# zz990099/foundationpose_cpp

Measured on AMD Instinct MI355X. Metric: pose-hypotheses/sec (Register N=252, 640x480), higher is better.
Workload: dtype f16; 1 GPU; Register N=252 hypotheses, 640x480 refine_itr=1, frame resident in HBM; mesh=synthetic ellipsoid V=2562 F=5120, 512x512 texture, weights=synthetic (seed 7), precision=f16 storage / f32 accumulate (the reference's TensorRT --fp16), parallelism=single GPU, collective=none

## Files before the change

### foundationpose_cpp_amd/csrc/fp_nn.hip

```cpp
#include "fp_nn.h"

#include <cmath>
#include <cstdio>
#include <cstdlib>
#include <cstring>
#include <algorithm>
#include <map>
#include <atomic>
#include <memory>
#include <thread>
#include <utility>

namespace fp {

typedef _Float16 h8 __attribute__((ext_vector_type(8)));
typedef _Float16 h4 __attribute__((ext_vector_type(4)));
typedef __bf16 b8 __attribute__((ext_vector_type(8)));
typedef __bf16 b4 __attribute__((ext_vector_type(4)));
typedef float f4 __attribute__((ext_vector_type(4)));
typedef int i2 __attribute__((ext_vector_type(2)));
typedef int i4 __attribute__((ext_vector_type(4)));
typedef int i8 __attribute__((ext_vector_type(8)));

static constexpr int EMBED = 512, HEADS = 4, HDIM = 128;
// ... 1034 lines not shown
  return 0;
}


struct Ctx {
  hipStream_t s;
  Profiler *prof;
  const Net *net;
  NNScratch *ws = nullptr;
};

#ifdef FP_TEST_HOOKS
#define FP_HOOK static int
static unsigned long long *g_clk_probe = nullptr;
static NNScratch g_hook_ws;
#else
#define FP_HOOK [[maybe_unused]] static constexpr int
static constexpr unsigned long long *g_clk_probe = nullptr;
#endif
FP_HOOK g_conv_variant = 0;
FP_HOOK g_conv_ablate = 0;
FP_HOOK g_splitk_ablate = 0;
FP_HOOK g_i8_stream = 0;
FP_HOOK g_smallm = 1;
FP_HOOK g_enc_tail = 1;
FP_HOOK g_ln_pmean = 1;
FP_HOOK g_fuse_pose = 1;
FP_HOOK g_qkv_ablate = 0;
FP_HOOK g_att_variant = 1;

static constexpr int SPLITK_TARGET = 128;
static constexpr int SPLITK_MIN_KT = 9;
static constexpr int SMALL_DEEP_MAXKT = 18;
static constexpr int SMALLM_MAXKT = 80;
static constexpr int SMALLM_MAXT16 = 1024;


enum ConvKernel {
  CK_SMALLX, CK_SMALLM, CK_STEM_HALO, CK_GEMM_K32, CK_S2_HALO, CK_HALO, CK_HALO8, CK_PP32, CK_BIG_PP, CK_PP, CK_DEEP64, CK_DEEP128,
  CK_IGEMM128, CK_IGEMM64, CK_SPLITK_REDUCE
};

struct ConvProblem {
  int Cin = 0, Cout = 0, KH = 0, KW = 0, stride = 1, pad = 0, algo_K = 0;
  bool wfrag = false, wpack = false;
  int NB = 0, H = 0, W = 0, ipad = 0;
  int dt = DT_F16, odt = DT_F16;
  bool has_res = false;
  int split_imgs = 0;
  int grp_rows = 0;
  bool post = false;
  int conv_variant = 0, conv_ablate = 0, smallm = 1;
};

struct ConvStep {
  int kernel = 0;
  const char *name = "";
  int mi = 0, ni = 0;
  bool post = false;
  bool deep = false;
  bool wpack = false;
  int ablate = 0;
  int m_begin = 0, M = 0;
  int ksplit = 1, kt_per = 0;
  unsigned grid = 0;
  int block = 256, lds = 0;
  double flops = 0, bytes = 0;
};

struct ConvPlan {
  static constexpr int MAX_STEPS = 4;
  int n = 0;
  ConvStep step[MAX_STEPS];
  bool post_fused = false;
};

static void conv_out_hw(int KH, int KW, int stride, int pad, int H, int W, int *OH, int *OW) {
  *OH = (H + 2 * pad - KH) / stride + 1;
  *OW = (W + 2 * pad - KW) / stride + 1;
  if (KH == 4 && pad == 2 && stride == 1) { *OH = H; *OW = W; }
}

static int plan_conv(const ConvProblem &q, ConvPlan *plan) {
  *plan = ConvPlan{};
  const bool B2 = !is_q8(q.dt);
  const bool SAME = q.dt == q.odt;
  const bool QOUT = odt_q(q.odt) >= 0;
  const bool grp = q.grp_rows > 0;
  int OH, OW;
  conv_out_hw(q.KH, q.KW, q.stride, q.pad, q.H, q.W, &OH, &OW);
  const int M = q.NB * OH * OW, Ktot = q.KH * q.KW * q.Cin, Cout = q.Cout;
  const int cin_b = q.Cin * elem_bytes(q.dt), KT = Ktot * elem_bytes(q.dt) / 128;
  double flops = 2.0 * (double)M * Cout * (q.algo_K > 0 ? q.algo_K : Ktot);
  double bytes = ((double)q.NB * q.H * q.W * q.Cin + (double)M * Cout * (q.has_res ? 2 : 1) + (double)Cout * Ktot) * elem_bytes(q.dt);
  constexpr int LDS_IG128 = 2 * (128 * 128 + 128 * 128), LDS_IG64 = 2 * (128 * 128 + 64 * 128);
  constexpr int LDS3_128 = 3 * (256 * 128 + 128 * 128);
  constexpr int LDS_BIG = 2 * (256 * 128 + 256 * 128);
  constexpr int LDS_HALO40 = ((10 * 42 + 7) / 8) * 1024 + 3 * 128 * 64;
  constexpr int LDS_HALO8 = ((10 * 42 + 7) / 8) * 1024 + 128 * 128;
  constexpr int LDS_STEM_HALO = ((11 * 84 + 15) / 16) * 1024 + 3 * 64 * 64;
  constexpr int LDS_DEEP64 = 6 * (64 + 128) * 128, LDS_DEEP128 = 4 * (128 + 128) * 128;
  constexpr int LDS_GEMM_K32 = 3 * (128 + 256) * 64;
  constexpr int LDS_S2_HALO = ((9 * 41 + 7) / 8) * 1024 + 3 * 128 * 64;
  constexpr int LDS_PP32 = 4 * (512 + 128) * 64;
  int m_begin = 0, ksplit = 1, kt_per = KT;
  bool overflow = false;
  const auto add = [&](int kernel, const char *name, int m_end, int grid, int block, int lds, double frac = 1.0) -> ConvStep & {
    overflow = overflow || plan->n == ConvPlan::MAX_STEPS;
    ConvStep &st = plan->step[overflow ? ConvPlan::MAX_STEPS - 1 : plan->n++];
    st = ConvStep{};
    st.kernel = kernel; st.name = name;
    st.m_begin = m_begin; st.M = m_end; st.ksplit = ksplit; st.kt_per = kt_per;
    st.grid = (unsigned)grid; st.block = block; st.lds = lds;
    st.flops = flops * frac; st.bytes = bytes * frac;
    flops *= (1.0 - frac); bytes *= (1.0 - frac);
    return st;
  };
  const auto finish = [&]() {
    FP_CHECK(!overflow, "plan_conv: more steps than ConvPlan holds");
    return 0;
// ... 54 lines not shown
      const int a = q.conv_ablate;
      add(CK_HALO, "conv_halo_kernel", M, grid, 256, LDS_HALO40).ablate = (q.dt == DT_F16 && (a == 1 || a == 2 || a == 8 || a == 16 || a == 32)) ? a : 0;
    } else {
      add(CK_HALO8, "conv_halo8_kernel", M, grid, 256, LDS_HALO8);
    }
    return finish();
  }
  if (B2 && !grp && (q.conv_variant == 0 || q.conv_variant == 8) && Cout == 128 && ksplit == 1 && KT >= 4 && KT <= 80) {
    const int mt_big = (M / 512 / 256) * 256;
    if (mt_big > 0) {
      add(CK_PP32, "conv_pp32_kernel<512,128>", mt_big * 512, mt_big, 512, LDS_PP32, (double)(mt_big * 512) / (double)M);
      m_begin = mt_big * 512;
      if (m_begin >= M) return finish();
    }
  }
  bool post_main = false;
  if (!(q.dt == DT_F16 && QOUT) && !grp && (q.conv_variant == 5 || q.conv_variant == 0 || q.conv_variant == 8) && Cout % 256 == 0 && ksplit == 1 && KT >= 2) {
    const int nt2 = Cout / 256;
    const int mt_all = M / 256;
    const int mt_big = (mt_all * nt2 / 256) * 256 / nt2;
    const int rows_left = M - mt_big * 256;
    post_main = q.post && !QOUT && mt_big > 0 && q.conv_variant == 0 && q.conv_ablate == 0 && KT >= 16 &&
                (rows_left == 0 || ((rows_left + 63) / 64) * (Cout / 128) <= 256);
    if (mt_big > 0) {
      const int a = q.conv_ablate;
      ConvStep &st = add(CK_BIG_PP, "conv_big_pp_kernel", mt_big * 256, mt_big * nt2, 512, LDS_BIG, (double)(mt_big * 256) / (double)M);
      st.ablate = (q.dt == DT_F16 && (a == 1 || a == 2 || a == 3 || a == 4 || a == 8 || a == 16)) ? a : 0;
      st.post = post_main;
      m_begin = mt_big * 256;
      if (m_begin >= M) { plan->post_fused = post_main; return finish(); }
    }
  }
  plan->post_fused = q.post && (post_main || ksplit > 1);
  if (!grp && (m_begin > 0 || M >= 8192 || small_deep) && (KT >= 16 || small_deep) && ksplit == 1 && Cout % 128 == 0) {
    const int n128 = Cout / 128;
    int rows = M - m_begin;
    if (((rows + 63) / 64) * n128 > 256) {
      const int mt_pp = (((rows + 255) / 256) * n128 / 256) * 256 / n128;
      const int rows_pp = std::min(mt_pp * 256, rows);
      const int rest = rows - rows_pp;
      const bool cascade = mt_pp > 0 && ((rest + 63) / 64) * n128 <= 256;
      const int m_end = cascade ? m_begin + rows_pp : M;
      add(CK_PP, "conv_pp_kernel(rem)", m_end, ((m_end - m_begin + 255) / 256) * n128, 512, LDS3_128, cascade ? (double)rows_pp / rows : 1.0);
      if (!cascade || rest == 0) return finish();
      m_begin += rows_pp;
      rows = rest;
// ... 445 lines not shown
  p.grp_rows = grp ? grp->rows : 0;
  p.in_shared = grp && grp->in_shared;
  p.res_shared = grp && grp->res_shared;
  p.grp_w_bytes = grp ? (unsigned)((size_t)L.Cout * L.KH * L.KW * L.Cin * es) : 0;
  FP_CHECK(!grp || (grp->rows % 128 == 0 && L.KH == 1 && L.KW == 1 && NB == 2 * grp->rows && !is_q8(L.dt)), "grouped launch: unsupported shape");
  p.in = (const unsigned char *)in.p; p.w = L.w; p.wfrag = L.wfrag; p.wpack = L.wpack; p.wpack128 = L.wpack128; p.wdeep = L.wdeep; p.bias = L.bias; p.cscale = is_q8(L.dt) ? L.cscale : nullptr;
  p.res = res ? (const unsigned char *)res->p : nullptr; p.out = (unsigned char *)out.p;
  p.out_dt = out.dt; p.res_dt = res ? res->dt : out.dt;
  p.NB = NB; p.H = H; p.W = W; p.Cin = L.Cin;
  p.KH = L.KH; p.KW = L.KW; p.stride = L.stride; p.pad = L.pad;
  p.ipad = ipad; p.opad = opad; p.rpad = rpad;
  conv_out_hw(L.KH, L.KW, L.stride, L.pad, H, W, &p.OH, &p.OW);
  p.Cout = L.Cout;
  p.M = NB * p.OH * p.OW;
  p.Ktot = L.KH * L.KW * L.Cin;
  p.cin_b = L.Cin * es;
  p.krow_b = p.Ktot * es;
  p.ntaps = L.KH * L.KW;
  p.relu = relu ? 1 : 0;
  p.split_imgs = split_imgs;
  p.out_ld = split_imgs > 0 ? 2 * L.Cout : L.Cout;
  p.res_ld = L.Cout;
  p.ksplit = 1; p.kt_per = p.krow_b / 128; p.partial = nullptr;
  p.m_begin = 0;
  FP_CHECK(ipad >= L.pad && (p.cin_b == 64 || p.cin_b % 128 == 0) && p.krow_b % 128 == 0 && (L.Cout % 64) == 0 &&
               (p.cin_b != 64 || L.KW % 2 == 0) && p.krow_b / 128 <= 80,
           "conv shape not supported by the MFMA kernel");
  {
    const int IWp = W + 2 * ipad;
    for (int kt = 0; kt < p.krow_b / 128; kt++) {
      int kh, kw, ch;
      if (p.cin_b >= 128) { ch = kt / p.ntaps; int tap = kt % p.ntaps; kh = tap / L.KW; kw = tap % L.KW; }
      else { ch = 0; int tap = 2 * kt; kh = tap / L.KW; kw = tap % L.KW; }
      p.koff[kt] = (unsigned)((kh * IWp + kw) * p.cin_b + ch * 128);
      if (2 * kt + 1 < 160) { p.koff32[2 * kt] = p.koff[kt]; p.koff32[2 * kt + 1] = p.koff[kt] + 64; }
    }
  }
  FP_CHECK(!res || res->dt == (rscale ? DT_I8 : is_q8(L.dt) ? DT_F16 : L.dt), "run_conv: the residual must have the layer's operand type (f16 for the 8-bit layers)");
  FP_CHECK(!post || (opad == 0 && split_imgs == 0 && !is_q8(out.dt) && post_fused), "run_conv: positional table on an unsupported layer");

  int odt = -1;
  ConvLaunch launch = nullptr;
#define FP_CONV_PAIR(DT_, ODT_) (odt = ODT_, launch = &launch_conv_step<DT_, ODT_>)
  if (out2) {
    if (L.dt == DT_FP8 && out2->dt == DT_FP8) FP_CONV_PAIR(DT_FP8, DT_DUAL_FP8);
    else if (L.dt == DT_I8 && out2->dt == DT_I8) FP_CONV_PAIR(DT_I8, DT_DUAL_I8);
    else if (L.dt == DT_F16 && out2->dt == DT_FP8) FP_CONV_PAIR(DT_F16, DT_DUAL_FP8);
// ... 12 lines not shown
      FP_CONV_PAIR(DT_F16, DT_QS_I8);
#else
      FP_CHECK(false, "run_conv: f16 -> scaled 8-bit alone exists in the test build only");
#endif
    } else FP_CONV_PAIR(DT_I8, DT_QS_I8);
  }
  else if (L.dt == DT_FP8 && out.dt == DT_FP8) FP_CONV_PAIR(DT_FP8, DT_FP8);
  else if (L.dt == DT_FP8 && out.dt == DT_F16) FP_CONV_PAIR(DT_FP8, DT_F16);
  else if (L.dt == DT_I8 && out.dt == DT_I8) FP_CONV_PAIR(DT_I8, DT_I8);
  else if (L.dt == DT_I8 && out.dt == DT_F16) FP_CONV_PAIR(DT_I8, DT_F16);
  else if (L.dt == DT_BF16 && out.dt == DT_BF16) FP_CONV_PAIR(DT_BF16, DT_BF16);
  else if (L.dt == DT_F16 && out.dt == DT_F16) FP_CONV_PAIR(DT_F16, DT_F16);
#undef FP_CONV_PAIR
  FP_CHECK(launch, "run_conv: unsupported combination of operand / output element types");

  ConvProblem q;
  q.Cin = L.Cin; q.Cout = L.Cout; q.KH = L.KH; q.KW = L.KW; q.stride = L.stride; q.pad = L.pad; q.algo_K = L.algo_K;
  q.wfrag = L.wfrag != nullptr; q.wpack = L.wpack != nullptr;
  q.NB = NB; q.H = H; q.W = W; q.ipad = ipad;
  q.dt = L.dt; q.odt = odt;
  q.has_res = res != nullptr; q.split_imgs = split_imgs;
  q.grp_rows = grp ? grp->rows : 0;
  q.post = post != nullptr;
  q.conv_variant = g_conv_variant; q.conv_ablate = g_conv_ablate; q.smallm = g_smallm;
  ConvPlan plan;
  if (plan_conv(q, &plan)) return 1;
  if (post_fused) *post_fused = plan.post_fused;
#ifdef FP_TEST_HOOKS
  g_last_conv_plan = plan; g_last_conv_odt = odt;
#endif
  for (int i = 0; i < plan.n; i++) {
    const ConvStep &st = plan.step[i];
    p.m_begin = st.m_begin; p.M = st.M;
    p.ksplit = st.ksplit; p.kt_per = st.kt_per;
    p.post = st.post ? (const unsigned char *)post : nullptr;
    if (st.ksplit > 1 && ensure_splitk(c, (size_t)st.ksplit * (st.M - st.m_begin) * L.Cout, &p.partial)) return 1;
    NetScope ps(c, tag, st);
    if (launch(c, st, p)) return 1;
  }
  return 0;
}

static int run_gemm(const Ctx &c, const char *tag, const ConvLayer &L, const void *in, int rows, void *out, bool relu,
                    const void *res = nullptr, const ConvGroup *grp = nullptr) {
  Act ai{const_cast<void *>(in), L.dt, 1.f}, ao{out, L.dt, 1.f}, ar{const_cast<void *>(res), L.dt, 1.f};
  return run_conv(c, tag, L, ai, rows, 1, 1, 0, ao, 0, relu, res ? &ar : nullptr, 0, 0, grp);
}

template <int DT>
struct DtTag {
  static constexpr int value = DT;
  using E = typename ElemT<DT>::t;
};
template <typename F>
static void with_dt(int dt, F &&f) {
  if (dt == DT_BF16) f(DtTag<DT_BF16>{});
// ... 718 lines not shown
```

### foundationpose_cpp_amd/csrc/fp_nn_conv_kernels.inc

```


__device__ __forceinline__ void glds16_asm(const void *gsrc, unsigned lds_addr) {
  unsigned keep;
  asm volatile("s_mov_b32 %0, m0\n\ts_mov_b32 m0, %2\n\ts_nop 0\n\tglobal_load_lds_dwordx4 %1, off\n\ts_mov_b32 m0, %0"
               : "=&s"(keep)
               : "v"(gsrc), "s"(lds_addr)
               : "memory");
}
__device__ __forceinline__ void glds16x2_asm(const void *gsrc, unsigned lds_addr) {
  unsigned keep;
  asm volatile("s_mov_b32 %0, m0\n\ts_mov_b32 m0, %2\n\ts_nop 0\n\tglobal_load_lds_dwordx4 %1, off\n\tglobal_load_lds_dwordx4 %1, off offset:1024\n\ts_mov_b32 m0, %0"
               : "=&s"(keep)
               : "v"(gsrc), "s"(lds_addr)
               : "memory");
}
__device__ __forceinline__ void glds16x4_asm(const void *gsrc, unsigned lds_addr) {
  unsigned keep;
  asm volatile("s_mov_b32 %0, m0\n\ts_mov_b32 m0, %2\n\ts_nop 0\n\tglobal_load_lds_dwordx4 %1, off\n\tglobal_load_lds_dwordx4 %1, off offset:1024\n\t"
               "global_load_lds_dwordx4 %1, off offset:2048\n\tglobal_load_lds_dwordx4 %1, off offset:3072\n\ts_mov_b32 m0, %0"
               : "=&s"(keep)
               : "v"(gsrc), "s"(lds_addr)
               : "memory");
}
#ifndef FP_X_NT
// ... 16 lines not shown
  const unsigned char *w;
  const unsigned char *wfrag;
  const unsigned char *wpack;
  const unsigned char *wpack128;
  const unsigned char *wdeep;
  const float *bias;
  const float *bias_img;
  const float *cscale;
  const unsigned char *res;
  unsigned char *out;
  unsigned char *out2;
  const float *rscale;
  const float *oinv;
  int NB, H, W, Cin, OH, OW, Cout, KH, KW, stride, pad;
  int ipad, opad, rpad;
  int M, Ktot, relu, out_ld, res_ld, split_imgs;
  int cin_b;
  int krow_b;
  int out_dt, res_dt;
  int ntaps;
  unsigned koff[80];
  unsigned koff32[160];
  int m_begin;
  int ksplit, kt_per;
  float *partial;
  int grp_rows, in_shared, res_shared;
  unsigned grp_w_bytes;
  unsigned long long *clk;
  const unsigned char *post;
};

__device__ __forceinline__ int pack4_fp8(float a, float b, float c, float d) {
  int w = __builtin_amdgcn_cvt_pk_fp8_f32(sat_fp8(a), sat_fp8(b), 0, false);
  return __builtin_amdgcn_cvt_pk_fp8_f32(sat_fp8(c), sat_fp8(d), w, true);
}
__device__ __forceinline__ int pack4_u8(float a, float b, float c, float d) {
  unsigned w = __builtin_amdgcn_cvt_pk_u8_f32(__builtin_rintf(a), 0, 0u);
  w = __builtin_amdgcn_cvt_pk_u8_f32(__builtin_rintf(b), 1, w);
  w = __builtin_amdgcn_cvt_pk_u8_f32(__builtin_rintf(c), 2, w);
  w = __builtin_amdgcn_cvt_pk_u8_f32(__builtin_rintf(d), 3, w);
  return (int)(w ^ 0x80808080u);
}
template <int MI, int NI, int DT, int ODT, int EABL = 0, int NIT = NI, int NI0 = 0, class PixFn>
__device__ __forceinline__ void conv_epilogue_px(const ConvParams &p, f4 (&acc)[NIT][MI], int n_base, int lane, PixFn pix,
                                                 int bias_off = 0, int res_img_off = 0) {
  static_assert(NI == 4 || NI == 2, "wave covers 64 or 32 channels");
// ... 12 lines not shown
    float4 b0 = *reinterpret_cast<const float4 *>(p.bias + bias_off + nl + 32 * k), b1 = *reinterpret_cast<const float4 *>(p.bias + bias_off + nl + 32 * k + 4);
    bv[0] = b0.x; bv[1] = b0.y; bv[2] = b0.z; bv[3] = b0.w; bv[4] = b1.x; bv[5] = b1.y; bv[6] = b1.z; bv[7] = b1.w;
    if constexpr (DT == DT_I8) {
      if (p.bias_img) {
#pragma unroll
        for (int e = 0; e < 8; e++) bv[e] = 0.f;
      }
    }
    if constexpr (is_q8(DT)) {
      float4 s0 = *reinterpret_cast<const float4 *>(p.cscale + bias_off + nl + 32 * k), s1 = *reinterpret_cast<const float4 *>(p.cscale + bias_off + nl + 32 * k + 4);
      sc[0] = s0.x; sc[1] = s0.y; sc[2] = s0.z; sc[3] = s0.w; sc[4] = s1.x; sc[5] = s1.y; sc[6] = s1.z; sc[7] = s1.w;
    }
#pragma unroll
    for (int e = 0; e < 8; e++) {
      const int jj = (NI == 4) ? 2 * k + (e >> 2) : (e >> 1);
      const int ni = (NI == 4) ? (e & 3) : (e & 1);
#pragma unroll
      for (int mi = 0; mi < MI; mi++) {
        if constexpr (DT == DT_I8) acc[NI0 + ni][mi][jj] = __builtin_fmaf((float)__float_as_int(acc[NI0 + ni][mi][jj]), sc[e], bv[e]);
        else if constexpr (DT == DT_FP8) acc[NI0 + ni][mi][jj] = __builtin_fmaf(acc[NI0 + ni][mi][jj], sc[e], bv[e]);
        else acc[NI0 + ni][mi][jj] += bv[e];
      }
    }
  }
  float oi[SCALED ? NS : 1][8];
  if constexpr (SCALED) {
#pragma unroll
    for (int k = 0; k < NS; k++) {
      float4 s0 = *reinterpret_cast<const float4 *>(p.oinv + nl + 32 * k), s1 = *reinterpret_cast<const float4 *>(p.oinv + nl + 32 * k + 4);
      oi[k][0] = s0.x; oi[k][1] = s0.y; oi[k][2] = s0.z; oi[k][3] = s0.w; oi[k][4] = s1.x; oi[k][5] = s1.y; oi[k][6] = s1.z; oi[k][7] = s1.w;
    }
  }
  float rs[RQ ? NS : 1][8];
  if constexpr (RQ) {
#pragma unroll
    for (int k = 0; k < NS; k++) {
      float4 s0 = *reinterpret_cast<const float4 *>(p.rscale + nl + 32 * k), s1 = *reinterpret_cast<const float4 *>(p.rscale + nl + 32 * k + 4);
      rs[k][0] = s0.x; rs[k][1] = s0.y; rs[k][2] = s0.z; rs[k][3] = s0.w; rs[k][4] = s1.x; rs[k][5] = s1.y; rs[k][6] = s1.z; rs[k][7] = s1.w;
    }
  }
  constexpr bool POST = (EABL & 4) != 0;
  static_assert(!POST || (O16 >= 0 && !DUAL), "the positional table is added to plain 2-byte outputs");
  constexpr int GB = (POST || is_q8(DT)) ? (MI > 4 ? 4 : MI) : (MI > 8 ? (MI + 1) / 2 : MI);
#pragma unroll
  for (int g0 = 0; g0 < MI; g0 += GB) {
  size_t oofs[GB];
// ... 702 lines not shown
  } else {
    for (int kt = 0; kt < KT; kt++) {
      if (kt > 0) mfmas();
      FP_PP_BARRIER();
      ldfrags(rb);
      if (kt + 2 < KT) {
        stage(kt + 2, wb3);
        asm volatile("s_waitcnt vmcnt(%0)" ::"n"(G) : "memory");
      } else {
        asm volatile("s_waitcnt vmcnt(0)" ::: "memory");
      }
      asm volatile("s_waitcnt lgkmcnt(0)" ::: "memory");
      FP_PP_BARRIER();
      rb = (rb == 2) ? 0 : rb + 1;
      wb3 = (wb3 == 2) ? 0 : wb3 + 1;
    }
    mfmas();
  }
#undef FP_PP_BARRIER

  conv_epilogue<4, NREP, DT, ODT>(p, acc, m0 + grp * 128 + wm * 64, n0 + wn * (BN / 2), lane);
}

template <int ABL, int DT, int ODT = DT, bool POST = false, bool LSTORE = false>
__global__ __launch_bounds__(512, 2) void conv_big_pp_kernel(const ConvParams p) {
  extern __shared__ __attribute__((aligned(16))) unsigned char smem[];
  constexpr int BM = 256, BN = 256;
  constexpr int XB = BM * 128, WB = BN * 128, STAGE = XB + WB;
  constexpr int MI = 8, NI = 4;

  const int tid = threadIdx.x, lane = tid & 63;
  const int wave = __builtin_amdgcn_readfirstlane(tid >> 6);
  const int wm = wave >> 2, wn = wave & 3;
  const int n_tiles = p.Cout / BN;
  int logical;
  {
    const int nblk = gridDim.x, b = blockIdx.x;
    const int xcd = b & 7, within = b >> 3, q = nblk >> 3, r = nblk & 7;
    logical = (xcd < r ? xcd * (q + 1) : r * (q + 1) + (xcd - r) * q) + within;
  }
  const int mt = logical / n_tiles, nt = logical - mt * n_tiles;
  const int m0 = mt * BM, n0 = nt * BN;
  const int ohw = p.OH * p.OW;
  const int IHp = p.H + 2 * p.ipad, IWp = p.W + 2 * p.ipad;

  const int srow = lane >> 3;
  const int g = (lane & 7) ^ srow;
  unsigned xoff[4], woffv[4];
#pragma unroll
  for (int i = 0; i < 4; i++) {
    int m = min(m0 + (wave * 4 + i) * 8 + srow, p.M - 1);
    int img = m / ohw;
    int rem = m - img * ohw;
    int oh = rem / p.OW, ow = rem - oh * p.OW;
    int ih0 = oh * p.stride - p.pad + p.ipad, iw0 = ow * p.stride - p.pad + p.ipad;
    xoff[i] = (unsigned)(((img * IHp + ih0) * IWp + iw0) * p.cin_b + g * 16);
    int row = (wave * 4 + i) * 8 + srow;
    woffv[i] = (unsigned)((n0 + row) * p.krow_b + g * 16);
  }
  const unsigned char *in_b = p.in;
  const unsigned char *w_b = p.w;
  const unsigned lds_base = (unsigned)(size_t)(__attribute__((address_space(3))) unsigned char *)smem;

  auto stage_x = [&](int kt, int buf) {
    const unsigned xs = lds_base + buf * STAGE;
    const unsigned char *xb = in_b + p.koff[kt];
#pragma unroll
    for (int i = 0; i < 4; i++) glds16_asm(xb + xoff[i], xs + (wave * 4 + i) * 1024);
  };
  const bool packed = p.wpack128 != nullptr;
  const unsigned char *wpk = p.wpack128 + ((size_t)nt * (p.krow_b >> 7) * 8 + wave) * 4096 + lane * 16;
  auto stage_w = [&](int kt, int buf) {
    const unsigned ws = lds_base + buf * STAGE + XB;
    if (packed) { glds16x4_asm(wpk + (size_t)kt * 32768, ws + wave * 4096); return; }
    const unsigned char *wb = w_b + (size_t)kt * 128;
#pragma unroll
    for (int i = 0; i < 4; i++) glds16_asm(wb + woffv[i], ws + (wave * 4 + i) * 1024);
  };

  f4 acc[NI][MI];
#pragma unroll
  for (int a = 0; a < NI; a++)
#pragma unroll
    for (int b = 0; b < MI; b++) acc[a][b] = (f4){0.f, 0.f, 0.f, 0.f};

  const int frow = lane & 15, fk = lane >> 4;
  int xfo[2], wfo[2];
#pragma unroll
  for (int ks = 0; ks < 2; ks++) {
    int slot = (ks * 4 + fk) ^ (lane & 7);
    xfo[ks] = (wm * 128 + frow) * 128 + slot * 16;
    wfo[ks] = XB + (wn * 64 + frow) * 128 + slot * 16;
  }

#define FP_BAR()                         \
  do {                                   \
    __builtin_amdgcn_s_barrier();        \
    asm volatile("" ::: "memory");      \
    __builtin_amdgcn_sched_barrier(0);   \
  } while (0)
#define FP_LGKM0() asm volatile("s_waitcnt lgkmcnt(0)" ::: "memory")
#define FP_VM0() asm volatile("s_waitcnt vmcnt(0)" ::: "memory")
#define FP_PP_LOOP(LD0, LD1, MF0, MF1)                                   \
  do {                                                                   \
    const int KT = p.krow_b >> 7;                                        \
    stage_x(0, 0);                                                       \
    stage_w(0, 0);                                                       \
    FP_VM0();                                                            \
    FP_BAR();                                                            \
    if (p.clk && tid == 0) { p.clk[blockIdx.x * 4] = __builtin_readcyclecounter(); p.clk[blockIdx.x * 4 + 1] = wall_clock64(); } \
    int buf = 0;                                                         \
    if (wm == 0) {                                                       \
      for (int kt = 0; kt < KT; kt++) {                                  \
        LD0(buf);                                                        \
// ... 80 lines not shown
      __builtin_amdgcn_s_setprio(1);
#pragma unroll
      for (int ni = 0; ni < NI; ni++)
#pragma unroll
        for (int mi = 0; mi < MI; mi++)
          acc[ni][mi] = mfma32<DT>(wf[ni], xf[mi], acc[ni][mi]);
      __builtin_amdgcn_s_setprio(0);
    };
    FP_PP_LOOP(ld0, ld1, mf, mf);
  }
#undef FP_PP_LOOP
#undef FP_BAR
#undef FP_LGKM0
#undef FP_VM0
  if (p.clk && tid == 0) { p.clk[blockIdx.x * 4 + 2] = __builtin_readcyclecounter(); p.clk[blockIdx.x * 4 + 3] = wall_clock64(); }

  if (ABL & 4) {
#pragma unroll
    for (int a = 0; a < NI; a++)
#pragma unroll
      for (int b = 0; b < MI; b++) asm volatile("" ::"v"(acc[a][b]));
    return;
  }
  if constexpr (LSTORE && ABL == 0 && !POST && !is_q8(DT) && odt_q(ODT) < 0) {
    __syncthreads();
    conv_epilogue_lds<MI, NI, DT, ODT, 4>(p, acc, m0 + wm * 128, n0 + wn * 64, lane, smem + wave * (4 * 16 * 128 + 4 * 64));
    return;
  }
  conv_epilogue<MI, NI, DT, ODT, ((ABL >> 3) & 3) | (POST ? 4 : 0)>(p, acc, m0 + wm * 128, n0 + wn * 64, lane);
}

template <int BM, int BN, int DT, int ODT = DT>
__global__ __launch_bounds__(512, 2) void conv_pp32_kernel(const ConvParams p) {
  extern __shared__ __attribute__((aligned(16))) unsigned char smem[];
  constexpr int WM = BM / 128, WN = BN / 64;
  static_assert(WM * WN == 8, "8 waves");
  constexpr int XP = BM / 16, WP = BN / 16, PER = (XP + WP) / 8;
  constexpr int XB = XP * 1024, STAGE = (XP + WP) * 1024;
  constexpr int MI = 8, NI = 4;

  const int tid = threadIdx.x, lane = tid & 63;
  const int wave = __builtin_amdgcn_readfirstlane(tid >> 6);
  const int grp = wave >> 2;
  const int wm = wave / WN, wn = wave - wm * WN;
  const int n_tiles = p.Cout / BN;
  int logical;
  {
    const int nblk = gridDim.x, b = blockIdx.x;
    const int xcd = b & 7, within = b >> 3, q = nblk >> 3, r = nblk & 7;
    logical = (xcd < r ? xcd * (q + 1) : r * (q + 1) + (xcd - r) * q) + within;
  }
  const int mt = logical / n_tiles, nt = logical - mt * n_tiles;
// ... 985 lines not shown
```

### foundationpose_cpp_amd/csrc/fp_nn_test_hooks.inc

```

__global__ __launch_bounds__(256) void mfma_peak_kernel(float *out, int iters, int zero_operands, unsigned long long *clk) {
  using fp::f4;
  using fp::h8;
  const int lane = threadIdx.x & 63;
  h8 a, b;
  unsigned st = 2654435761u * (unsigned)(blockIdx.x * 256 + threadIdx.x + 1);
#pragma unroll
  for (int i = 0; i < 8; i++) {
    st = st * 1664525u + 1013904223u;
    a[i] = (_Float16)(((st >> 8) & 0xffff) / 65536.0f - 0.5f);
    st = st * 1664525u + 1013904223u;
    b[i] = (_Float16)(((st >> 8) & 0xffff) / 65536.0f - 0.5f);
    if (zero_operands) { a[i] = 0; b[i] = 0; }
  }
  unsigned long long c0 = 0, w0 = 0;
  if (clk && blockIdx.x == 0 && threadIdx.x == 0) { c0 = __builtin_readcyclecounter(); w0 = wall_clock64(); }
  f4 acc[8];
#pragma unroll
  for (int j = 0; j < 8; j++) acc[j] = (f4){0.f, 0.f, 0.f, 0.f};
  for (int i = 0; i < iters; i++) {
#pragma unroll
    for (int j = 0; j < 8; j++)
      asm volatile("v_mfma_f32_16x16x32_f16 %0, %1, %2, %0" : "+v"(acc[j]) : "v"(a), "v"(b));
  }
// ... 90 lines not shown
  fp::ConvLayer L;
  L.Cout = Cout; L.Cin = Cin; L.ntaps = ntaps;
  L.rows_f32.assign(rows, rows + (size_t)Cout * ntaps * Cin);
  std::vector<float> sw, tm;
  std::vector<double> qsum;
  const auto q = fp::quantise_q8(L, fp::DT_I8, s_in, &sw, &qsum, m_int, J, &tm);
  std::memcpy(q_out, q.data(), q.size());
  std::memcpy(sw_out, sw.data(), sw.size() * sizeof(float));
  std::memcpy(tmat_t_out, tm.data(), tm.size() * sizeof(float));
  return 0;
}
int fpt_quantise_q8(int dt, const float *rows, int Cout, int ntaps, int Cin, const float *s_in, unsigned char *q_out, float *sw_out) {
  if (!fp::is_q8(dt) || !rows || !s_in || !q_out || !sw_out || Cout < 1 || ntaps < 1 || Cin < 1) return 1;
  fp::ConvLayer L;
  L.Cout = Cout; L.Cin = Cin; L.ntaps = ntaps;
  L.rows_f32.assign(rows, rows + (size_t)Cout * ntaps * Cin);
  std::vector<float> sw;
  std::vector<double> qsum;
  const auto q = fp::quantise_q8(L, dt, s_in, &sw, &qsum);
  std::memcpy(q_out, q.data(), q.size());
  std::memcpy(sw_out, sw.data(), sw.size() * sizeof(float));
  return 0;
}
int fpt_plan_conv(const int *shape10, int dt, int odt, int flags, int split_imgs, int grp_rows, int *fields11, char *names, int name_cap, int max, int *post_fused) {
  fp::ConvProblem q;
  q.Cin = shape10[0]; q.Cout = shape10[1]; q.KH = shape10[2]; q.KW = shape10[3]; q.stride = shape10[4]; q.pad = shape10[5];
  q.NB = shape10[6]; q.H = shape10[7]; q.W = shape10[8]; q.ipad = shape10[9];
  q.dt = dt; q.odt = odt;
  q.has_res = (flags & 1) != 0; q.post = (flags & 2) != 0; q.wfrag = (flags & 4) != 0; q.wpack = (flags & 8) != 0;
  q.split_imgs = split_imgs; q.grp_rows = grp_rows;
  q.conv_variant = fp::g_conv_variant; q.conv_ablate = fp::g_conv_ablate; q.smallm = fp::g_smallm;
  fp::ConvPlan plan;
  if (fp::plan_conv(q, &plan)) return -1;
  for (int i = 0; i < plan.n && i < max; i++) {
    const fp::ConvStep &st = plan.step[i];
    const int f[11] = {-1, -1, 0, st.m_begin, st.M, st.ksplit, st.post ? 1 : 0, st.kernel, st.kt_per, (int)st.grid, st.lds};
    std::memcpy(fields11 + (size_t)i * 11, f, sizeof(f));
    std::snprintf(names + (size_t)i * name_cap, (size_t)name_cap, "%s", st.name);
  }
  if (post_fused) *post_fused = plan.post_fused ? 1 : 0;
  return plan.n;
}
int fpt_plan_heads(int pass, int N, int dt, int fuse_offer, int *fields18, int *tail3) {
  fp::HeadsPlan p;
  if (fp::plan_heads(fp::heads_query(pass, N, dt, fuse_offer != 0), &p)) return 1;
  const fp::AttVariant &v = fp::ATT_VARIANTS[p.att.variant];
  const int f[18] = {p.qkv, p.qkv_ablate, (int)p.qkv_grid, p.qkv_lds, p.att.kernel, v.remap ? 1 : 0, v.ablate, p.att.B, p.att.T,
                     p.att.pitch, p.att.nq, (int)p.att.grid, p.att.block, p.att.lds, p.tail, p.pool, p.readout, p.fuse_pose ? 1 : 0};
  std::memcpy(fields18, f, sizeof(f));
  const int t[3] = {p.tail_tiles, (int)p.tail_grid, p.tail_lds};
  std::memcpy(tail3, t, sizeof(t));
  return 0;
}
void fpt_plan_track_window(const float *K9, float diameter, const float *poses16, int H, int W, int reach, int *out5, int n) {
  for (int i = 0; i < n; i++) {
    const fp::TrackWindow w = fp::plan_track_window(K9, diameter, poses16 + (size_t)i * 16, H, W, reach);
    const int f[5] = {w.kind, w.row0, w.row1, w.col0, w.col1};
    for (int k = 0; k < 5; k++) out5[(size_t)i * 5 + k] = f[k];
  }
}
void fpt_depth_filter_tile(int *tile_w, int *tile_h) { *tile_w = fp::DEPTH_FILTER_TILE_W; *tile_h = fp::DEPTH_FILTER_TILE_H; }
void fpt_set_conv_variant(int v) { fp::g_conv_variant = v; }
void fpt_set_i8_stream(int v) { fp::g_i8_stream = v; }
void fpt_set_q8_blocks(int v) { fp::g_q8_blocks = v & fp::Q8_BLOCKS_ALL; }
void fpt_set_conv_ablate(int v) { fp::g_conv_ablate = v; }
void fpt_set_splitk_ablate(int v) { fp::g_splitk_ablate = v; }

int fpt_clk_probe(int blocks, double *mhz_out, double *loop_cycles_out) {
  using namespace fp;
  if (blocks > 0) {
    if (g_clk_probe) (void)hipFree(g_clk_probe);
    FP_HIP_OK(hipMalloc((void **)&g_clk_probe, (size_t)blocks * 32));
    FP_HIP_OK(fp::memset_sync(g_clk_probe, 0, (size_t)blocks * 32));
    return 0;
  }
  FP_CHECK(g_clk_probe, "no probe");
  int n = -blocks;
  std::vector<unsigned long long> h((size_t)n * 4);
  FP_HIP_OK(hipDeviceSynchronize());
  FP_HIP_OK(fp::memcpy_sync(h.data(), g_clk_probe, h.size() * 8, hipMemcpyDeviceToHost));
  double sc = 0, sr = 0; int cnt = 0;
  for (int i = 0; i < n; i++) {
    if (h[i * 4 + 3] > h[i * 4 + 1]) { sc += (double)(h[i * 4 + 2] - h[i * 4]); sr += (double)(h[i * 4 + 3] - h[i * 4 + 1]); cnt++; }
  }
  if (mhz_out) *mhz_out = sr > 0 ? sc / sr * 100.0 : 0;
  if (loop_cycles_out) *loop_cycles_out = cnt ? sc / cnt : 0;
  (void)hipFree(g_clk_probe);
  g_clk_probe = nullptr;
  return 0;
}

int fpt_conv_dt(const float *x, const float *w, const float *bias, const float *res, int NB, int H, int W, int Cin, int Cout,
                int KH, int KW, int stride, int pad, int OH, int OW, int relu, int split_imgs, float *out, int iters,
                float *ms_out, int dt, int out_dt, float in_scale, float res_scale, float out_scale) {
  using namespace fp;
  const int ip = pad;
  const int Hp = H + 2 * ip, Wp = W + 2 * ip;
  const int es = elem_bytes(dt), oes = elem_bytes(out_dt);
  size_t nx = (size_t)NB * Hp * Wp * Cin, nw = (size_t)Cout * KH * KW * Cin;
  size_t M = (size_t)NB * OH * OW;
  size_t nout = M * Cout;
  DevBuf<unsigned char> dx(nx * es), dres(nout * es), dout(nout * 2 * oes);
  FP_CHECK(dx.p && dres.p && dout.p, "fpt_conv: allocation failed");
  std::vector<float> xp(nx, 0.f);
  for (int n = 0; n < NB; n++)
    for (int y = 0; y < H; y++)
      for (int xx = 0; xx < W; xx++)
        for (int c = 0; c < Cin; c++)
          xp[(((size_t)n * Hp + y + ip) * Wp + xx + ip) * Cin + c] = x[(((size_t)n * H + y) * W + xx) * Cin + c];
  auto hx = encode(xp.data(), nx, dt, in_scale);
  FP_HIP_OK(fp::memcpy_sync(dx.p, hx.data(), hx.size(), hipMemcpyHostToDevice));
  FP_HIP_OK(fp::memset_sync(dout.p, 0, nout * 2 * oes));
  if (res) {
    auto hr = encode(res, nout, dt, res_scale);
    FP_HIP_OK(fp::memcpy_sync(dres.p, hr.data(), hr.size(), hipMemcpyHostToDevice));
  }
  Net net;
  ConvLayer L;
  L.Cin = Cin; L.Cout = Cout; L.KH = KH; L.KW = KW; L.stride = stride; L.pad = pad;
  FP_CHECK(finish_layer(&net, std::vector<float>(w, w + nw), std::vector<float>(bias, bias + Cout), Cout, KH * KW, Cin, dt, &L), "fpt_conv: weight upload failed");
  FP_CHECK(!is_q8(dt) && !is_q8(out_dt), "fpt_conv_dt: 2-byte element types only (8-bit layers: fpt_conv_q8)");
  Ctx c{nullptr, nullptr, &net};
  (void)OH; (void)OW;
  const Act ain{dx.p, dt, in_scale}, aout{dout.p, out_dt, out_scale}, ares{dres.p, dt, res_scale};
  hipEvent_t e0, e1;
  FP_HIP_OK(hipEventCreate(&e0));
  FP_HIP_OK(hipEventCreate(&e1));
  if (run_conv(c, "t", L, ain, NB, H, W, ip, aout, 0, relu != 0, res ? &ares : nullptr, 0, split_imgs)) return 1;
  FP_HIP_OK(hipDeviceSynchronize());
  if (iters > 1) {
    FP_HIP_OK(hipEventRecord(e0, nullptr));
    for (int i = 0; i < iters; i++)
      if (run_conv(c, "t", L, ain, NB, H, W, ip, aout, 0, relu != 0, res ? &ares : nullptr, 0, split_imgs)) return 1;
    FP_HIP_OK(hipEventRecord(e1, nullptr));
    FP_HIP_OK(hipEventSynchronize(e1));
    float ms = 0;
    FP_HIP_OK(hipEventElapsedTime(&ms, e0, e1));
    if (ms_out) *ms_out = ms / iters;
  }
  (void)hipEventDestroy(e0);
  (void)hipEventDestroy(e1);
  std::vector<unsigned char> ho(nout * oes);
  FP_HIP_OK(fp::memcpy_sync(ho.data(), dout.p, ho.size(), hipMemcpyDeviceToHost));
  decode(ho.data(), nout, out_dt, out_scale, out);
  return 0;
}
int fpt_conv_q8(const float *x, const float *s_in, const float *w, const float *bias, const float *res, int NB, int H, int W, int Cin, int Cout,
                int KH, int KW, int stride, int pad, int OH, int OW, int relu, int split_imgs, int mode, const float *s_out, float *out16,
                float *outq, int iters, float *ms_out, int dt, float *wq_out, const float *s_res) {
  using namespace fp;
  FP_CHECK(is_q8(dt) && mode >= 0 && mode <= 5 && (mode < 4 || (dt == DT_I8 && res && s_res)), "fpt_conv_q8: invalid arguments");
  const int ip = pad, Hp = H + 2 * ip, Wp = W + 2 * ip;
  const size_t nx = (size_t)NB * Hp * Wp * Cin, nw = (size_t)Cout * KH * KW * Cin, M = (size_t)NB * OH * OW, nout = M * Cout;
  DevBuf<unsigned char> dx(nx), dres(nout * 2), d16(nout * 2), dq(nout);
  FP_CHECK(dx.p && dres.p && d16.p && dq.p, "fpt_conv_q8: allocation failed");
  std::vector<unsigned char> hx(nx, dt == DT_I8 ? 0x80 : 0x00);
  for (int n = 0; n < NB; n++)
    for (int y = 0; y < H; y++)
      for (int xx = 0; xx < W; xx++)
        for (int c = 0; c < Cin; c++) {
          const float v = x[(((size_t)n * H + y) * W + xx) * Cin + c] / s_in[c];
          unsigned char b;
          if (dt == DT_FP8) b = f32_to_e4m3_bits(v);
          else b = (unsigned char)((int)std::max(0.f, std::min(255.f, std::nearbyint(v))) ^ 0x80);
          hx[(((size_t)n * Hp + y + ip) * Wp + xx + ip) * Cin + c] = b;
        }
  FP_HIP_OK(fp::memcpy_sync(dx.p, hx.data(), nx, hipMemcpyHostToDevice));
// ... 637 lines not shown
```

Before: 23930 hypotheses/s.

## Absorb conv big-tile row remainder into taller 288-row tiles instead of a tail launch

When the big 256x256 conv path leaves leftover rows, the planner now spreads them over some blocks that use a 288-row (MI=9) tile, each taking an extra 32 rows, balanced across XCDs. The whole convolution then runs as one launch instead of a main kernel plus a separate tail kernel. The kernel body is templated on MI, and a ragged epilogue handles the partial tile. This adds LDS per block and register pressure for the tall variant, and the test harness gains guard bands to catch out-of-bounds writes.

```diff
diff --git a/foundationpose_cpp_amd/csrc/fp_nn.hip b/foundationpose_cpp_amd/csrc/fp_nn.hip
--- a/foundationpose_cpp_amd/csrc/fp_nn.hip
+++ b/foundationpose_cpp_amd/csrc/fp_nn.hip
@@ -1080,6 +1080,7 @@
 FP_HOOK g_conv_ablate = 0;
 FP_HOOK g_splitk_ablate = 0;
 FP_HOOK g_i8_stream = 0;
+FP_HOOK g_conv_ragged = 1;
 FP_HOOK g_smallm = 1;
 FP_HOOK g_enc_tail = 1;
 FP_HOOK g_ln_pmean = 1;
@@ -1109,6 +1110,7 @@
   int grp_rows = 0;
   bool post = false;
   int conv_variant = 0, conv_ablate = 0, smallm = 1;
+  int ragged = 1;
 };
 
 struct ConvStep {
@@ -1120,6 +1122,7 @@
   bool wpack = false;
   int ablate = 0;
   int m_begin = 0, M = 0;
+  int n_tall = 0;
   int ksplit = 1, kt_per = 0;
   unsigned grid = 0;
   int block = 256, lds = 0;
@@ -1154,6 +1157,7 @@
   constexpr int LDS_IG128 = 2 * (128 * 128 + 128 * 128), LDS_IG64 = 2 * (128 * 128 + 64 * 128);
   constexpr int LDS3_128 = 3 * (256 * 128 + 128 * 128);
   constexpr int LDS_BIG = 2 * (256 * 128 + 256 * 128);
+  constexpr int LDS_BIG_TALL = 2 * (288 * 128 + 256 * 128);
   constexpr int LDS_HALO40 = ((10 * 42 + 7) / 8) * 1024 + 3 * 128 * 64;
   constexpr int LDS_HALO8 = ((10 * 42 + 7) / 8) * 1024 + 128 * 128;
   constexpr int LDS_STEM_HALO = ((11 * 84 + 15) / 16) * 1024 + 3 * 64 * 64;
@@ -1254,6 +1258,12 @@
     const int rows_left = M - mt_big * 256;
     post_main = q.post && !QOUT && mt_big > 0 && q.conv_variant == 0 && q.conv_ablate == 0 && KT >= 16 &&
                 (rows_left == 0 || ((rows_left + 63) / 64) * (Cout / 128) <= 256);
+    const int n_tall = (rows_left + 31) / 32;
+    if (q.ragged && B2 && SAME && mt_big > 0 && rows_left > 0 && q.conv_variant == 0 && q.conv_ablate == 0 && !q.post && 256 % nt2 == 0 &&
+        n_tall * nt2 <= 256) {
+      add(CK_BIG_PP, "conv_big_pp_kernel", M, mt_big * nt2, 512, LDS_BIG_TALL).n_tall = n_tall;
+      return finish();
+    }
     if (mt_big > 0) {
       const int a = q.conv_ablate;
       ConvStep &st = add(CK_BIG_PP, "conv_big_pp_kernel", mt_big * 256, mt_big * nt2, 512, LDS_BIG, (double)(mt_big * 256) / (double)M);
@@ -1745,7 +1755,7 @@
   p.out_ld = split_imgs > 0 ? 2 * L.Cout : L.Cout;
   p.res_ld = L.Cout;
   p.ksplit = 1; p.kt_per = p.krow_b / 128; p.partial = nullptr;
-  p.m_begin = 0;
+  p.m_begin = 0; p.n_tall = 0;
   FP_CHECK(ipad >= L.pad && (p.cin_b == 64 || p.cin_b % 128 == 0) && p.krow_b % 128 == 0 && (L.Cout % 64) == 0 &&
                (p.cin_b != 64 || L.KW % 2 == 0) && p.krow_b / 128 <= 80,
            "conv shape not supported by the MFMA kernel");
@@ -1804,7 +1814,7 @@
   q.has_res = res != nullptr; q.split_imgs = split_imgs;
   q.grp_rows = grp ? grp->rows : 0;
   q.post = post != nullptr;
-  q.conv_variant = g_conv_variant; q.conv_ablate = g_conv_ablate; q.smallm = g_smallm;
+  q.conv_variant = g_conv_variant; q.conv_ablate = g_conv_ablate; q.smallm = g_smallm; q.ragged = g_conv_ragged;
   ConvPlan plan;
   if (plan_conv(q, &plan)) return 1;
   if (post_fused) *post_fused = plan.post_fused;
@@ -1813,7 +1823,7 @@
 #endif
   for (int i = 0; i < plan.n; i++) {
     const ConvStep &st = plan.step[i];
-    p.m_begin = st.m_begin; p.M = st.M;
+    p.m_begin = st.m_begin; p.M = st.M; p.n_tall = st.n_tall;
     p.ksplit = st.ksplit; p.kt_per = st.kt_per;
     p.post = st.post ? (const unsigned char *)post : nullptr;
     if (st.ksplit > 1 && ensure_splitk(c, (size_t)st.ksplit * (st.M - st.m_begin) * L.Cout, &p.partial)) return 1;
diff --git a/foundationpose_cpp_amd/csrc/fp_nn_conv_kernels.inc b/foundationpose_cpp_amd/csrc/fp_nn_conv_kernels.inc
--- a/foundationpose_cpp_amd/csrc/fp_nn_conv_kernels.inc
+++ b/foundationpose_cpp_amd/csrc/fp_nn_conv_kernels.inc
@@ -62,6 +62,7 @@
   unsigned koff[80];
   unsigned koff32[160];
   int m_begin;
+  int n_tall;
   int ksplit, kt_per;
   float *partial;
   int grp_rows, in_shared, res_shared;
@@ -120,6 +121,12 @@
         else acc[NI0 + ni][mi][jj] += bv[e];
       }
     }
+  }
+  if constexpr ((EABL & 8) != 0) {
+#pragma unroll
+    for (int a = 0; a < NI; a++)
+#pragma unroll
+      for (int b = 0; b < MI; b++) asm volatile("" : "+v"(acc[NI0 + a][b]));
   }
   float oi[SCALED ? NS : 1][8];
   if constexpr (SCALED) {
@@ -868,39 +875,35 @@
   conv_epilogue<4, NREP, DT, ODT>(p, acc, m0 + grp * 128 + wm * 64, n0 + wn * (BN / 2), lane);
 }
 
-template <int ABL, int DT, int ODT = DT, bool POST = false, bool LSTORE = false>
-__global__ __launch_bounds__(512, 2) void conv_big_pp_kernel(const ConvParams p) {
-  extern __shared__ __attribute__((aligned(16))) unsigned char smem[];
-  constexpr int BM = 256, BN = 256;
+template <int MI, int ABL, int DT, int ODT, bool POST, bool LSTORE>
+__device__ __forceinline__ void conv_big_pp_body(const ConvParams &p, unsigned char *smem, const int m0, const int nt) {
+  constexpr int BM = MI * 32, BN = 256;
   constexpr int XB = BM * 128, WB = BN * 128, STAGE = XB + WB;
-  constexpr int MI = 8, NI = 4;
+  constexpr int NI = 4;
+  constexpr int NPX = BM / 8, PLO = NPX / 8, PREM = NPX % 8, PHI = PLO + (PREM ? 1 : 0);
 
   const int tid = threadIdx.x, lane = tid & 63;
   const int wave = __builtin_amdgcn_readfirstlane(tid >> 6);
   const int wm = wave >> 2, wn = wave & 3;
-  const int n_tiles = p.Cout / BN;
-  int logical;
-  {
-    const int nblk = gridDim.x, b = blockIdx.x;
-    const int xcd = b & 7, within = b >> 3, q = nblk >> 3, r = nblk & 7;
-    logical = (xcd < r ? xcd * (q + 1) : r * (q + 1) + (xcd - r) * q) + within;
-  }
-  const int mt = logical / n_tiles, nt = logical - mt * n_tiles;
-  const int m0 = mt * BM, n0 = nt * BN;
+  const int n0 = nt * BN;
   const int ohw = p.OH * p.OW;
   const int IHp = p.H + 2 * p.ipad, IWp = p.W + 2 * p.ipad;
 
   const int srow = lane >> 3;
   const int g = (lane & 7) ^ srow;
-  unsigned xoff[4], woffv[4];
-#pragma unroll
-  for (int i = 0; i < 4; i++) {
-    int m = min(m0 + (wave * 4 + i) * 8 + srow, p.M - 1);
+  const int px0 = wave * PLO + min(wave, PREM);
+  unsigned xoff[PHI], woffv[4];
+#pragma unroll
+  for (int i = 0; i < PHI; i++) {
+    int m = min(m0 + (px0 + i) * 8 + srow, p.M - 1);
     int img = m / ohw;
     int rem = m - img * ohw;
     int oh = rem / p.OW, ow = rem - oh * p.OW;
     int ih0 = oh * p.stride - p.pad + p.ipad, iw0 = ow * p.stride - p.pad + p.ipad;
     xoff[i] = (unsigned)(((img * IHp + ih0) * IWp + iw0) * p.cin_b + g * 16);
+  }
+#pragma unroll
+  for (int i = 0; i < 4; i++) {
     int row = (wave * 4 + i) * 8 + srow;
     woffv[i] = (unsigned)((n0 + row) * p.krow_b + g * 16);
   }
@@ -912,7 +915,8 @@
     const unsigned xs = lds_base + buf * STAGE;
     const unsigned char *xb = in_b + p.koff[kt];
 #pragma unroll
-    for (int i = 0; i < 4; i++) glds16_asm(xb + xoff[i], xs + (wave * 4 + i) * 1024);
+    for (int i = 0; i < PHI; i++)
+      if (i < PLO || wave < PREM) glds16_asm(xb + xoff[i], xs + (px0 + i) * 1024);
   };
   const bool packed = p.wpack128 != nullptr;
   const unsigned char *wpk = p.wpack128 + ((size_t)nt * (p.krow_b >> 7) * 8 + wave) * 4096 + lane * 16;
@@ -935,7 +939,7 @@
 #pragma unroll
   for (int ks = 0; ks < 2; ks++) {
     int slot = (ks * 4 + fk) ^ (lane & 7);
-    xfo[ks] = (wm * 128 + frow) * 128 + slot * 16;
+    xfo[ks] = (wm * (MI * 16) + frow) * 128 + slot * 16;
     wfo[ks] = XB + (wn * 64 + frow) * 128 + slot * 16;
   }
 
@@ -1062,12 +1066,38 @@
       for (int b = 0; b < MI; b++) asm volatile("" ::"v"(acc[a][b]));
     return;
   }
-  if constexpr (LSTORE && ABL == 0 && !POST && !is_q8(DT) && odt_q(ODT) < 0) {
+  if constexpr (LSTORE && MI == 8 && ABL == 0 && !POST && !is_q8(DT) && odt_q(ODT) < 0) {
     __syncthreads();
     conv_epilogue_lds<MI, NI, DT, ODT, 4>(p, acc, m0 + wm * 128, n0 + wn * 64, lane, smem + wave * (4 * 16 * 128 + 4 * 64));
     return;
   }
-  conv_epilogue<MI, NI, DT, ODT, ((ABL >> 3) & 3) | (POST ? 4 : 0)>(p, acc, m0 + wm * 128, n0 + wn * 64, lane);
+  constexpr bool RAGGED = ABL == 0 && !POST && !LSTORE && !is_q8(DT) && odt_q(ODT) < 0;
+  conv_epilogue<MI, NI, DT, ODT, ((ABL >> 3) & 3) | (POST ? 4 : 0) | (RAGGED ? 8 : 0)>(p, acc, m0 + wm * (MI * 16), n0 + wn * 64, lane);
+}
+
+template <int ABL, int DT, int ODT = DT, bool POST = false, bool LSTORE = false>
+__global__ __launch_bounds__(512, 2) void conv_big_pp_kernel(const ConvParams p) {
+  extern __shared__ __attribute__((aligned(16))) unsigned char smem[];
+  constexpr bool RAGGED = ABL == 0 && !POST && !LSTORE && !is_q8(DT) && odt_q(ODT) < 0;
+  const int n_tiles = p.Cout / 256;
+  const int nblk = gridDim.x, b = blockIdx.x;
+  const int xcd = b & 7, within = b >> 3, q = nblk >> 3, r = nblk & 7;
+  const int logical = (xcd < r ? xcd * (q + 1) : r * (q + 1) + (xcd - r) * q) + within;
+  const int mt = logical / n_tiles, nt = logical - mt * n_tiles;
+  int m0 = p.m_begin + mt * 256;
+  if constexpr (RAGGED) {
+    if (p.n_tall > 0) {
+      const int tq = p.n_tall >> 3, tr = p.n_tall & 7;
+      const int t_x = tq + (xcd < tr ? 1 : 0);
+      const int lt = within / n_tiles;
+      m0 += 32 * (xcd * tq + min(xcd, tr) + min(lt, t_x));
+      if (lt < t_x) {
+        conv_big_pp_body<9, ABL, DT, ODT, POST, LSTORE>(p, smem, m0, nt);
+        return;
+      }
+    }
+  }
+  conv_big_pp_body<8, ABL, DT, ODT, POST, LSTORE>(p, smem, m0, nt);
 }
 
 template <int BM, int BN, int DT, int ODT = DT>
diff --git a/foundationpose_cpp_amd/csrc/fp_nn_test_hooks.inc b/foundationpose_cpp_amd/csrc/fp_nn_test_hooks.inc
--- a/foundationpose_cpp_amd/csrc/fp_nn_test_hooks.inc
+++ b/foundationpose_cpp_amd/csrc/fp_nn_test_hooks.inc
@@ -136,6 +136,8 @@
   std::memcpy(sw_out, sw.data(), sw.size() * sizeof(float));
   return 0;
 }
+static fp::ConvPlan g_hook_conv_plan;
+int fpt_plan_conv_tall(int i) { return i >= 0 && i < g_hook_conv_plan.n ? g_hook_conv_plan.step[i].n_tall : -1; }
 int fpt_plan_conv(const int *shape10, int dt, int odt, int flags, int split_imgs, int grp_rows, int *fields11, char *names, int name_cap, int max, int *post_fused) {
   fp::ConvProblem q;
   q.Cin = shape10[0]; q.Cout = shape10[1]; q.KH = shape10[2]; q.KW = shape10[3]; q.stride = shape10[4]; q.pad = shape10[5];
@@ -143,9 +145,11 @@
   q.dt = dt; q.odt = odt;
   q.has_res = (flags & 1) != 0; q.post = (flags & 2) != 0; q.wfrag = (flags & 4) != 0; q.wpack = (flags & 8) != 0;
   q.split_imgs = split_imgs; q.grp_rows = grp_rows;
-  q.conv_variant = fp::g_conv_variant; q.conv_ablate = fp::g_conv_ablate; q.smallm = fp::g_smallm;
+  q.conv_variant = fp::g_conv_variant; q.conv_ablate = fp::g_conv_ablate; q.smallm = fp::g_smallm; q.ragged = fp::g_conv_ragged;
   fp::ConvPlan plan;
+  g_hook_conv_plan = fp::ConvPlan{};
   if (fp::plan_conv(q, &plan)) return -1;
+  g_hook_conv_plan = plan;
   for (int i = 0; i < plan.n && i < max; i++) {
     const fp::ConvStep &st = plan.step[i];
     const int f[11] = {-1, -1, 0, st.m_begin, st.M, st.ksplit, st.post ? 1 : 0, st.kernel, st.kt_per, (int)st.grid, st.lds};
@@ -175,6 +179,7 @@
 }
 void fpt_depth_filter_tile(int *tile_w, int *tile_h) { *tile_w = fp::DEPTH_FILTER_TILE_W; *tile_h = fp::DEPTH_FILTER_TILE_H; }
 void fpt_set_conv_variant(int v) { fp::g_conv_variant = v; }
+void fpt_set_conv_ragged(int v) { fp::g_conv_ragged = v != 0; }
 void fpt_set_i8_stream(int v) { fp::g_i8_stream = v; }
 void fpt_set_q8_blocks(int v) { fp::g_q8_blocks = v & fp::Q8_BLOCKS_ALL; }
 void fpt_set_conv_ablate(int v) { fp::g_conv_ablate = v; }
@@ -204,6 +209,7 @@
   return 0;
 }
 
+static constexpr size_t CONV_DT_GUARD = 64 * 1024;
 int fpt_conv_dt(const float *x, const float *w, const float *bias, const float *res, int NB, int H, int W, int Cin, int Cout,
                 int KH, int KW, int stride, int pad, int OH, int OW, int relu, int split_imgs, float *out, int iters,
                 float *ms_out, int dt, int out_dt, float in_scale, float res_scale, float out_scale) {
@@ -214,8 +220,11 @@
   size_t nx = (size_t)NB * Hp * Wp * Cin, nw = (size_t)Cout * KH * KW * Cin;
   size_t M = (size_t)NB * OH * OW;
   size_t nout = M * Cout;
-  DevBuf<unsigned char> dx(nx * es), dres(nout * es), dout(nout * 2 * oes);
-  FP_CHECK(dx.p && dres.p && dout.p, "fpt_conv: allocation failed");
+  const size_t G = CONV_DT_GUARD;
+  DevBuf<unsigned char> dx(nx * es), dres(nout * es), dguard(nout * oes + 2 * G);
+  FP_CHECK(dx.p && dres.p && dguard.p, "fpt_conv: allocation failed");
+  struct { unsigned char *p; } dout{dguard.p + G};
+  FP_HIP_OK(fp::memset_sync(dguard.p, 0xA5, nout * oes + 2 * G));
   std::vector<float> xp(nx, 0.f);
   for (int n = 0; n < NB; n++)
     for (int y = 0; y < H; y++)
@@ -224,7 +233,7 @@
           xp[(((size_t)n * Hp + y + ip) * Wp + xx + ip) * Cin + c] = x[(((size_t)n * H + y) * W + xx) * Cin + c];
   auto hx = encode(xp.data(), nx, dt, in_scale);
   FP_HIP_OK(fp::memcpy_sync(dx.p, hx.data(), hx.size(), hipMemcpyHostToDevice));
-  FP_HIP_OK(fp::memset_sync(dout.p, 0, nout * 2 * oes));
+  FP_HIP_OK(fp::memset_sync(dout.p, 0, nout * oes));
   if (res) {
     auto hr = encode(res, nout, dt, res_scale);
     FP_HIP_OK(fp::memcpy_sync(dres.p, hr.data(), hr.size(), hipMemcpyHostToDevice));
@@ -257,6 +266,11 @@
   std::vector<unsigned char> ho(nout * oes);
   FP_HIP_OK(fp::memcpy_sync(ho.data(), dout.p, ho.size(), hipMemcpyDeviceToHost));
   decode(ho.data(), nout, out_dt, out_scale, out);
+  std::vector<unsigned char> hg(2 * G);
+  FP_HIP_OK(fp::memcpy_sync(hg.data(), dguard.p, G, hipMemcpyDeviceToHost));
+  FP_HIP_OK(fp::memcpy_sync(hg.data() + G, dout.p + nout * oes, G, hipMemcpyDeviceToHost));
+  for (unsigned char v : hg)
+    if (v != 0xA5) { fp::set_error("fpt_conv_dt: the kernels wrote outside the output buffer"); return 2; }
   return 0;
 }
 int fpt_conv_q8(const float *x, const float *s_in, const float *w, const float *bias, const float *res, int NB, int H, int W, int Cin, int Cout,
```

Measured after the change: 24480 hypotheses/s, median of 6. +2.3%, better.
